# zeahmed/NeuralASR

Measured on AMD Instinct MI355X. Metric: audio-frames/sec (fwd+bwd+CTC+Adam) at batch 16 per GPU, higher is better.
Workload: dtype f32

## Files before the change

### neuralasr_amd/csrc/gemm.hip

```cpp
#include "kernels.h"

namespace nasr {

typedef float f32x16 __attribute__((ext_vector_type(16)));

constexpr int BM = 128, BN = 128, BK = 16, LDT = 132;

struct GemmParams {
  const float* A;
  const float* B;
  float* C;
  int M, N, K, lda, ldb, ldc;
  const int* a_map;
  int a_shift, a_rows;
  const int* c_map;
  const float* bias;
  int split_k, kchunk;
  float* slabs;
};

__device__ __forceinline__ int phys_row(const int* map, int shift, int rows, int logical) {
  int r = map ? map[logical] : logical + shift;
  return (r >= 0 && r < rows) ? r : -1;
}

__device__ __forceinline__ float4 ld4(const float* __restrict__ p) { return *reinterpret_cast<const float4*>(p); }
__device__ __forceinline__ float4 sel4(bool ok, float4 v) {
  return make_float4(ok ? v.x : 0.f, ok ? v.y : 0.f, ok ? v.z : 0.f, ok ? v.w : 0.f);
}

template <bool ACOL, bool BCOL>
__global__ __launch_bounds__(256, 2) void gemm_kernel(GemmParams p) {
  __shared__ __attribute__((aligned(16))) float As[2][BK][LDT];
  __shared__ __attribute__((aligned(16))) float Bs[2][BK][LDT];
  const int tid = threadIdx.x, lane = tid & 63, w = tid >> 6;
  const int m0 = blockIdx.y * BM, n0 = blockIdx.x * BN;
  const int kbeg = blockIdx.z * p.kchunk;
  const int kend = min(p.K, kbeg + p.kchunk);
  const int nk = (kend - kbeg + BK - 1) / BK;
  const float* __restrict__ Ag = p.A;
  const float* __restrict__ Bg = p.B;

  constexpr int NS = BK / 8, KQ = BK / 4;
  bool aok[NS], bok[NS];
  size_t ao[NS], bo[NS];
#pragma unroll
  for (int j = 0; j < NS; ++j) {
    const int idx = tid + 256 * j;
    const int r = idx / KQ, kq = idx % KQ, q = idx & 31;
    if (!ACOL) {
      const int pa = (m0 + r < p.M) ? phys_row(p.a_map, p.a_shift, p.a_rows, m0 + r) : -1;
      aok[j] = pa >= 0;
      ao[j] = aok[j] ? (size_t)pa * p.lda + 4 * kq : 0;
    } else {
      aok[j] = (m0 + 4 * q < p.M);
      ao[j] = aok[j] ? (size_t)(m0 + 4 * q) : 0;
    }
    if (BCOL) {
      bok[j] = n0 + r < p.N;
      bo[j] = bok[j] ? (size_t)(n0 + r) * p.ldb + 4 * kq : 0;
    } else {
      bok[j] = (n0 + 4 * q < p.N);
      bo[j] = bok[j] ? (size_t)(n0 + 4 * q) : 0;
    }
  }

  float4 ra[NS], rb[NS];
#define NASR_GLOAD(K0)                                                                              \
  _Pragma("unroll") for (int j = 0; j < NS; ++j) {                                                  \
    const int kk_ = (tid + 256 * j) >> 5;                                                           \
    const bool kr_ = (K0) + 4 * ((tid + 256 * j) % KQ) < kend, kc_ = (K0) + kk_ < kend;             \
    if (!ACOL) {                                                                                    \
      const bool o_ = aok[j] && kr_;                                                                \
      ra[j] = sel4(o_, ld4(Ag + (o_ ? ao[j] + (K0) : 0)));                                          \
    } else {                                                                                        \
      const int pr_ = kc_ ? phys_row(p.a_map, p.a_shift, p.a_rows, (K0) + kk_) : -1;                \
      const bool o_ = aok[j] && pr_ >= 0;                                                           \
      ra[j] = sel4(o_, ld4(Ag + (o_ ? (size_t)pr_ * p.lda + ao[j] : 0)));                           \
    }                                                                                               \
    if (BCOL) {                                                                                     \
      const bool o_ = bok[j] && kr_;                                                                \
      rb[j] = sel4(o_, ld4(Bg + (o_ ? bo[j] + (K0) : 0)));                                          \
    } else {                                                                                        \
      const bool o_ = bok[j] && kc_;                                                                \
      rb[j] = sel4(o_, ld4(Bg + (o_ ? (size_t)((K0) + kk_) * p.ldb + bo[j] : 0)));                  \
    }                                                                                               \
  }
#define NASR_LSTORE(BUF)                                                                            \
  _Pragma("unroll") for (int j = 0; j < NS; ++j) {                                                  \
    const int idx_ = tid + 256 * j;                                                                 \
    const int r_ = idx_ / KQ, kq_ = idx_ % KQ, kk_ = idx_ >> 5, q_ = idx_ & 31;                     \
    if (!ACOL) {                                                                                    \
      As[BUF][4 * kq_ + 0][r_] = ra[j].x; As[BUF][4 * kq_ + 1][r_] = ra[j].y;                       \
      As[BUF][4 * kq_ + 2][r_] = ra[j].z; As[BUF][4 * kq_ + 3][r_] = ra[j].w;                       \
    } else {                                                                                        \
      *reinterpret_cast<float4*>(&As[BUF][kk_][4 * q_]) = ra[j];                                    \
    }                                                                                               \
    if (BCOL) {                                                                                     \
      Bs[BUF][4 * kq_ + 0][r_] = rb[j].x; Bs[BUF][4 * kq_ + 1][r_] = rb[j].y;                       \
      Bs[BUF][4 * kq_ + 2][r_] = rb[j].z; Bs[BUF][4 * kq_ + 3][r_] = rb[j].w;                       \
    } else {                                                                                        \
      *reinterpret_cast<float4*>(&Bs[BUF][kk_][4 * q_]) = rb[j];                                    \
    }                                                                                               \
  }

  f32x16 acc00, acc01, acc10, acc11;
#pragma unroll
  for (int r = 0; r < 16; ++r) { acc00[r] = 0.f; acc01[r] = 0.f; acc10[r] = 0.f; acc11[r] = 0.f; }

  const int wm = (w >> 1) * 64, wn = (w & 1) * 64;
  const int li = lane & 31, lk = lane >> 5;

  if (nk > 0) {
    NASR_GLOAD(kbeg);
    NASR_LSTORE(0);
  }
  __syncthreads();
  for (int kt = 0; kt < nk; ++kt) {
    const int buf = kt & 1;
    const bool more = kt + 1 < nk;
    if (more) NASR_GLOAD(kbeg + (kt + 1) * BK);
    float a0 = As[buf][lk][wm + li], a1 = As[buf][lk][wm + 32 + li];
    float b0 = Bs[buf][lk][wn + li], b1 = Bs[buf][lk][wn + 32 + li];
#pragma unroll
    for (int ks = 0; ks < BK / 2; ++ks) {
      float na0 = 0.f, na1 = 0.f, nb0 = 0.f, nb1 = 0.f;
      if (ks + 1 < BK / 2) {
        const int k = 2 * (ks + 1) + lk;
        na0 = As[buf][k][wm + li]; na1 = As[buf][k][wm + 32 + li];
        nb0 = Bs[buf][k][wn + li]; nb1 = Bs[buf][k][wn + 32 + li];
      }
      acc00 = __builtin_amdgcn_mfma_f32_32x32x2f32(a0, b0, acc00, 0, 0, 0);
      acc01 = __builtin_amdgcn_mfma_f32_32x32x2f32(a0, b1, acc01, 0, 0, 0);
      acc10 = __builtin_amdgcn_mfma_f32_32x32x2f32(a1, b0, acc10, 0, 0, 0);
      acc11 = __builtin_amdgcn_mfma_f32_32x32x2f32(a1, b1, acc11, 0, 0, 0);
      a0 = na0; a1 = na1; b0 = nb0; b1 = nb1;
    }
    if (more) NASR_LSTORE(buf ^ 1);
    __syncthreads();
  }
#undef NASR_GLOAD
#undef NASR_LSTORE

#pragma unroll
  for (int t = 0; t < 4; ++t) {
    const int mi = t >> 1, ni = t & 1;
    const f32x16 acc = t == 0 ? acc00 : t == 1 ? acc01 : t == 2 ? acc10 : acc11;
    const int col = n0 + wn + 32 * ni + li;
    if (col >= p.N) continue;
    const float bv = (p.bias && p.split_k == 1) ? p.bias[col] : 0.f;
#pragma unroll
    for (int r = 0; r < 16; ++r) {
      const int row = m0 + wm + 32 * mi + (r & 3) + 8 * (r >> 2) + 4 * lk;
      if (row >= p.M) continue;
      if (p.split_k > 1) {
        p.slabs[((size_t)blockIdx.z * p.M + row) * p.N + col] = acc[r];
      } else {
        const int pr = p.c_map ? p.c_map[row] : row;
        if (pr >= 0) p.C[(size_t)pr * p.ldc + col] = acc[r] + bv;
      }
    }
  }
}

__global__ __launch_bounds__(256) void gemm_reduce_kernel(GemmParams p) {
  const int64_t n4 = (int64_t)p.M * p.N / 4;
  for (int64_t i = blockIdx.x * (int64_t)blockDim.x + threadIdx.x; i < n4; i += (int64_t)gridDim.x * blockDim.x) {
    const int64_t e = i * 4;
    const int row = (int)(e / p.N), col = (int)(e % p.N);
    float4 s = *reinterpret_cast<const float4*>(p.slabs + e);
    for (int k = 1; k < p.split_k; ++k) {
      const float4 v = *reinterpret_cast<const float4*>(p.slabs + (size_t)k * p.M * p.N + e);
      s.x += v.x; s.y += v.y; s.z += v.z; s.w += v.w;
    }
    if (p.bias) { s.x += p.bias[col]; s.y += p.bias[col + 1]; s.z += p.bias[col + 2]; s.w += p.bias[col + 3]; }
    const int pr = p.c_map ? p.c_map[row] : row;
    if (pr >= 0) *reinterpret_cast<float4*>(p.C + (size_t)pr * p.ldc + col) = s;
  }
}

int gemm_pick_split(int M, int N, int K) {
  const int tiles = ((M + BM - 1) / BM) * ((N + BN - 1) / BN);
  int s = (512 + tiles - 1) / tiles;
  const int max_s = K / 128;
  if (s > max_s) s = max_s;
  if (s < 1) s = 1;
  return s;
}

void launch_gemm(const GemmDesc& g, hipStream_t st) {
  GemmParams p;
  p.A = g.A; p.B = g.B; p.C = g.C;
  p.M = g.M; p.N = g.N; p.K = g.K; p.lda = g.lda; p.ldb = g.ldb; p.ldc = g.ldc;
  p.a_map = g.a_map; p.a_shift = g.a_shift; p.a_rows = g.a_rows; p.c_map = g.c_map; p.bias = g.bias;
  p.split_k = g.split_k < 1 ? 1 : g.split_k;
  p.slabs = g.slabs;
  int kt = (g.K + BK - 1) / BK;
  int per = (kt + p.split_k - 1) / p.split_k;
  p.kchunk = per * BK;
  p.split_k = (kt + per - 1) / per;
  dim3 grid((g.N + BN - 1) / BN, (g.M + BM - 1) / BM, p.split_k), block(256);
  if (!g.a_col && !g.b_col) hipLaunchKernelGGL((gemm_kernel<false, false>), grid, block, 0, st, p);
  else if (g.a_col && !g.b_col) hipLaunchKernelGGL((gemm_kernel<true, false>), grid, block, 0, st, p);
  else if (!g.a_col && g.b_col) hipLaunchKernelGGL((gemm_kernel<false, true>), grid, block, 0, st, p);
  else hipLaunchKernelGGL((gemm_kernel<true, true>), grid, block, 0, st, p);
  if (p.split_k > 1) {
    int64_t n4 = (int64_t)g.M * g.N / 4;
    int blocks = (int)((n4 + 255) / 256);
    if (blocks > 2048) blocks = 2048;
    hipLaunchKernelGGL(gemm_reduce_kernel, dim3(blocks), dim3(256), 0, st, p);
  }
}

}
```

### neuralasr_amd/csrc/kernels.h

```cpp
#pragma once
#include <hip/hip_runtime.h>
#include <stdint.h>

namespace nasr {

const char* test_hook(const char* name);

struct GemmDesc {
  const float* A;
  const float* B;
  float* C;
  int M, N, K;
  int lda, ldb, ldc;
  bool a_col;
  bool b_col;
  const int* a_map;
  int a_shift;
  int a_rows;
  const int* c_map;
  const float* bias;
  int split_k;
  float* slabs;
};
void launch_gemm(const GemmDesc& g, hipStream_t st);
int gemm_pick_split(int M, int N, int K);

int tp_split2_parts(int rows);
int gemm_tp_tile_rows(int M);
size_t tph_bytes(int rows, int K);
size_t tph_scale_ws_floats(int rows, int K);
void launch_tph_scales(const float* src, int rows, int K, int ld, float* row_scale, float* row_inv, float* col_scale,
                       float* col_inv, float* ws, hipStream_t st);
constexpr int TPH_MAX_JOBS = 16;
struct TphScaleJob { const float* src; int rows, K, ld; float *row_scale, *row_inv, *col_scale, *col_inv; };
size_t tph_scale_batch_ws_floats(const TphScaleJob* jobs, int n);
void launch_tph_scales_batch(const TphScaleJob* jobs, int n, float* ws, hipStream_t st);
void launch_tph_scales_from_parts(const float* rowpart, int nrp, int rows, float* row_scale, float* row_inv, const float* colpart,
                                  int ncp, int K, float* col_scale, float* col_inv, hipStream_t st);
void launch_fill(float* p, float v, int n, hipStream_t st);
void launch_tph_split2(const float* src, unsigned char* tpN, unsigned char* tpT, int rows, int K, int ld,
                       const float* row_scale, float rs, const float* col_scale, float cs, float* colpart, hipStream_t st,
                       const int* rowmap = nullptr, const int* rowmap2 = nullptr, int col2 = 0);
void launch_gather_rows(float* dst, const float* src, const int* map, int n, float fill, hipStream_t st);
struct GemmTPHDesc {
  const unsigned char* A;
  const unsigned char* B;
  float* C;
  int M, N, K;
  int nkbA, nkbB;
  int ldc;
  int a_kshift;
  const float* bias;
  const float* a_inv;
  const float* b_inv;
  int split_k;
  float* slabs;
  int tile_rows;
  int nbatch;
  size_t a_bstride, b_bstride;
  int64_t c_bstride, ainv_bstride, binv_bstride;
  int a_kshift1;
  bool side;
  const int* c_map;
};
hipError_t gemm_tph_prepare();
int gemm_tph_pick_split(int M, int N, int K, int nbatch = 1);
void launch_gemm_tph(const GemmTPHDesc& g, hipStream_t st);

struct LstmDims { int T, B, Bp, H, Hp, D; };
void launch_repack_u(const float* U, float* Uf, float* Ub, int Hp, hipStream_t st);
int lstm_bwd_partials(int Hp);
struct StepWindow {
  LstmDims dm;
  const float *Uf, *Ub;
  float *hstate, *partial, *dcstate;
  float *gates, *cbuf, *out;
  float* dg;
  const float* dout;
  const int* seq_len;
  float forget_bias;
  const float* c0;
};
void lstm_steps_fwd(const StepWindow& w, int s0, int s1, hipStream_t st);
void lstm_steps_bwd(const StepWindow& w, int s0, int s1, hipStream_t st);
struct StepLeft { float *partial, *dc; };
float* lstm_steps_dcin(const StepWindow& w, int s);
StepLeft lstm_steps_left(const StepWindow& w, int s);
constexpr int LA_MAX_SLOTS = 64;
struct LaSlots { int held[LA_MAX_SLOTS], n[LA_MAX_SLOTS], emit[LA_MAX_SLOTS]; };
void launch_stream_load_state(const float* state, float* himg, float* cimg, int S, int H, int Bp, int Hp, hipStream_t st, int D = 1);
void launch_stream_save_state(const float* out, const float* cbuf, const LaSlots& sl, float* state, int S, int H, int Bp, int DH,
                              hipStream_t st);

struct LcGeom { int C, W, K, T, Bp; };
__host__ __device__ inline int lc_last_window(int len, int C, int W) { return len <= W ? 0 : (len - W + C - 1) / C; }
__host__ __device__ inline int lc_window_rows(int len, int k, int C, int W) {
  if (len < 1 || k > lc_last_window(len, C, W)) return 0;
  return len - k * C < W ? len - k * C : W;
}
void launch_lc_load_carry(const float* out, const float* cbuf, const int* wlen, int k, const LcGeom& g, float* himg, float* cimg,
                          int Hp, int D, hipStream_t st);
void launch_lc_carry_out(const float* part, int np, const float* dcs, const int* wlen_k, float* drow, float* dcc, int Bp, int Hp,
                         int DH, hipStream_t st);
void launch_lc_carry_dc(float* dcin, const float* dcc, int n, hipStream_t st);

void launch_pack_feats(const float* feats_bm, float* X0, int B, int Bp, int T, int F, int Fp, hipStream_t st);
void launch_expand_context(const float* centre, const float* pad, const int* seq_len, float* X0, int B, int Bp, int T,
                           int ctx, int ncep, int Fp, hipStream_t st);
void launch_expand_context_masked(const float* centre, const float* pad, const int* seq_len, const int* masks, int nm,
                                  int static_width, float* X0, int B, int Bp, int T, int ctx, int ncep, int Fp,
                                  hipStream_t st);
void launch_la_window(const float* hold_in, const float* fresh, const LaSlots& sl, float* win, float* hold_out, int S, int R,
                      int Tc, int T, int rows, int F, hipStream_t st);
void launch_lc_gather(const float* src, const int* wlen, float* dst, const LcGeom& g, int F, hipStream_t st);
void launch_lc_emit(const float* outv, const int* seq_len, float* top, const LcGeom& g, int DH, hipStream_t st);
void launch_lc_scatter(const float* dtop, const int* seq_len, const int* wlen, float* doutv, const LcGeom& g, int DH,
                       hipStream_t st);

struct XcdCtl {
  unsigned xcc_count[8];
  unsigned error;
  unsigned pad[23];
};
static_assert(sizeof(XcdCtl) == 32 * sizeof(unsigned), "the control blocks' head is 32 words");
struct PersistCtl : XcdCtl {
  unsigned flags[8 * 128];
#if defined(NASR_PSTAMP) && NASR_PSTAMP
  unsigned stamps[256][12];
#endif
};
bool persist_supported(int Hp);
size_t persist_image_floats(int Hp, bool bwd);
size_t persist_xch_floats(int Hp);
size_t persist_hx_bytes(int Hp);
size_t persist_px_bytes();
hipError_t persist_prepare();
constexpr int PERSIST_MAX_MATS = 16;
void launch_repack_persist(const float* P, const int64_t* offs, int n, float* Upf, float* Upb, int Hp, const float* col_scale,
                           hipStream_t st);
void launch_lstm_persist_fwd(const LstmDims& dm, const float* Upf, const float* cinv, float* gates, float* cbuf,
                             float* out, const int* seq_len, float* xch, PersistCtl* ctl, unsigned* sticky, float* fault,
                             float forget_bias, hipStream_t st, bool ctl_zeroed = false);
void launch_lstm_persist_bwd(const LstmDims& dm, const float* Upb, const float* gates, float* dgbuf, const float* cbuf,
                             const float* dout, const int* seq_len, float* xch, PersistCtl* ctl, unsigned* sticky,
                             float* fault, hipStream_t st, bool ctl_zeroed = false, float* rowpart = nullptr,
                             float* colpart = nullptr, bool lean = false);
size_t persist_dgmax_floats(int T, int Bp, int Hp, int D);

struct WideCtl : XcdCtl {
  unsigned stamps[160];
};
struct WideGeom {
  int T, Bp, Hp, D, d;
  int inject;
  int scale_shift;
  float* fault;
};
bool wide_supported(int Hp, int Bp);
size_t wide_image_bytes(int Hp);
size_t wide_hx_bytes(int Bp);
size_t wide_part_bytes(int Bp);
hipError_t wide_prepare();
void launch_repack_wide(const float* U, const float* cs, void* Uw, int Hp, hipStream_t st);
void launch_lstm_wide_fwd(const LstmDims& dm, int d, const void* Uw, const float* cinv, float* gates, float* cbuf,
                          float* out, const int* seq_len, void* hx, float* part, WideCtl* ctl, unsigned* sticky,
                          float* fault, float forget_bias, hipStream_t st);

size_t wide_px_bytes(int Bp);
void launch_repack_wide_bwd(const float* U, const float* rs, void* Uwb, int Hp, hipStream_t st);
void launch_wide_row_scales(const LstmDims& dm, const float* dout, const int* seq_len, float* srow, hipStream_t st);
void launch_lstm_wide_bwd(const LstmDims& dm, int d, const void* Uwb, const float* rinv, const float* srow,
                          const float* gates, float* dgbuf, const float* cbuf, const float* dout, const int* seq_len,
                          float* inbox, void* px, WideCtl* ctl, unsigned* sticky, float* fault, hipStream_t st);

void launch_dense_act(float* z, int R, int Bp, int B, int W, int ld, float clip, float p, uint32_t seed, uint32_t counter,
                      int stage, hipStream_t st);
void launch_dense_act_bwd(float* dy, const float* y, int64_t n, float clip, float p, hipStream_t st);

struct CtcDims {
  int Tp;
  int B, Bp, C, Cp, Lmax;
  int KS;
  int Tws;
  float* lprobs = nullptr;
  double* goff = nullptr;
};
constexpr int ctc_states_per_lane(int Lmax) {
  const int KS = (2 * (Lmax > 0 ? Lmax : 0) + 1 + 63) / 64;
  return KS <= 1 ? 2 : KS <= 8 ? KS : KS <= 12 ? 12 : KS <= 16 ? 16 : KS;
}
constexpr int ctc_group_rows(int Tws) { return Tws / 4 + 3; }
void launch_ctc_logz(const CtcDims& d, const float* logits, const int* seq_len, float* logz, hipStream_t st);
void launch_ctc_alpha_beta(const CtcDims& d, const float* logits, const float* logz, const int* labels,
                           const int* label_len, const int* seq_len, float* alpha, float* beta, double* aoff,
                           double* boff, float* nll, double* logp, hipStream_t st);
void launch_ctc_grad(const CtcDims& d, float* logits, const float* logz, const int* label_len, const int* seq_len,
                     const int* cstart, const int* cpos, const float* alpha, const float* beta, const double* aoff,
                     const double* boff, const double* logp, float scale, hipStream_t st);
void launch_mean(const float* v, int n, float* out, hipStream_t st);
void launch_greedy(const CtcDims& d, const float* logits, const int* seq_len, int* argmax_ws, int* ids, int* lens,
                   hipStream_t st);

bool ctc_align_bp_in_lds(int F, int L);
size_t ctc_align_ws_words(int B, int F, int L);
int launch_ctc_align(const CtcDims& d, int F, const float* logits, const float* logz, const int* labels, const int* label_len,
                     const int* seq_len, unsigned* bpws, int* path, double* score, hipStream_t st);

void launch_distill_rows(const CtcDims& d, const float* student, const float* teacher, const int* seq_len, float weight,
                         float tau, float* dgrad, float* klrow, double* kd, hipStream_t st);
void launch_distill_combine(const double* kd, int B, float weight, float tau, float* loss, float* parts,
                            const float* teacher_fault, float* fault, hipStream_t st);
void launch_distill_add(const CtcDims& d, float* grad, const float* dgrad, hipStream_t st);

struct AdamDev { long long step; float lr_t; int applied; };
struct EmaDev { long long updates; float omd; };
constexpr int ADAM_MAX_BLOCKS = 2048;
void launch_adam(float* p, float* m, float* v, const float* g, int64_t n, AdamDev* state, float lr, float beta1, float beta2,
                 float eps, float gscale, const float* fault, float* e, EmaDev* ema, float decay, hipStream_t st);
void launch_swap16(float* a, float* b, int64_t n, hipStream_t st);
struct ClipDev { double last_norm; float last_coef, s; int skip, pad; double window_max_norm; long long steps, clipped, skipped; };
constexpr int GRAD_SUMSQ_MAX_BLOCKS = 1024;
int grad_sumsq_blocks(int64_t n);
void launch_adam_clipped(float* p, float* m, float* v, const float* g, int64_t n, AdamDev* state, ClipDev* clip, double* part,
                         float lr, float beta1, float beta2, float eps, float gscale, float max_norm, const float* fault,
                         float* e, EmaDev* ema, float decay, hipStream_t st);
void launch_colsum(const float* M, int R, int N, int ld, float* out, float* ws, hipStream_t st);
void launch_colsum_parts(const float* part, int nparts, int N, float* out, hipStream_t st);
void launch_reduce_slabs(const float* slabs, int S, int64_t n, float* out, hipStream_t st);
void launch_reduce_slabs_rows(const float* slabs, int S, int M, int N, int ldc, const int* map, float* out, hipStream_t st);
void launch_ring_standin(float* buf, int64_t n, int nblocks, int passes, hipStream_t st);

}
```

### neuralasr_amd/csrc/optim.hip

```cpp
#include "kernels.h"

#include <cstdlib>

namespace nasr {

const char* test_hook(const char* name) {
  static const bool enabled = [] {
    const char* e = getenv("NASR_TEST_HOOKS");
    return e && e[0] == '1';
  }();
  return enabled ? getenv(name) : nullptr;
}

__device__ __forceinline__ void adam_advance(AdamDev* st, float lr, float b1, float b2) {
  const long long t = st->step + 1;
  st->step = t;
  st->lr_t = (float)((double)lr * sqrt(1.0 - pow((double)b2, (double)t)) / (1.0 - pow((double)b1, (double)t)));
  st->applied = 1;
}

__device__ __forceinline__ void ema_advance(EmaDev* em, float decay) {
  if (!em) return;
  const long long n = em->updates;
  const double ramp = (1.0 + (double)n) / (10.0 + (double)n);
  const double d = (double)decay < ramp ? (double)decay : ramp;
  em->omd = (float)(1.0 - d);
  em->updates = n + 1;
}

__global__ void adam_prepare_kernel(AdamDev* st, const float* __restrict__ fault, float lr, float b1, float b2, EmaDev* em,
                                    float decay) {
  if (fault && *fault != 0.f) {
    st->applied = 0;
    return;
  }
  adam_advance(st, lr, b1, b2);
  ema_advance(em, decay);
}

#define NASR_ADAM_SWEEP(EMA)                                                                                              \
  for (int64_t i = blockIdx.x * (int64_t)blockDim.x + threadIdx.x; i < n4; i += (int64_t)gridDim.x * blockDim.x) {       \
    float4 gg = reinterpret_cast<const float4*>(g)[i];                                                                    \
    float4 mm = reinterpret_cast<float4*>(m)[i];                                                                          \
    float4 vv = reinterpret_cast<float4*>(v)[i];                                                                          \
    float4 pp = reinterpret_cast<float4*>(p)[i];                                                                          \
    NASR_ADAM1(x) NASR_ADAM1(y) NASR_ADAM1(z) NASR_ADAM1(w)                                                               \
    reinterpret_cast<float4*>(m)[i] = mm;                                                                                 \
    reinterpret_cast<float4*>(v)[i] = vv;                                                                                 \
    reinterpret_cast<float4*>(p)[i] = pp;                                                                                 \
    NASR_EMA_##EMA                                                                                                        \
  }
#define NASR_EMA_0
#define NASR_EMA_1                                                                                                        \
  {                                                                                                                       \
    float4 ee = reinterpret_cast<float4*>(e)[i];                                                                          \
    ee.x = fmaf(omd, pp.x - ee.x, ee.x);                                                                                  \
    ee.y = fmaf(omd, pp.y - ee.y, ee.y);                                                                                  \
    ee.z = fmaf(omd, pp.z - ee.z, ee.z);                                                                                  \
    ee.w = fmaf(omd, pp.w - ee.w, ee.w);                                                                                  \
    reinterpret_cast<float4*>(e)[i] = ee;                                                                                 \
  }
#define NASR_ADAM1(c)                                   \
  {                                                     \
    const float gc = gg.c * gscale;                     \
    mm.c = b1 * mm.c + (1.f - b1) * gc;                 \
    vv.c = b2 * vv.c + (1.f - b2) * gc * gc;            \
    pp.c = pp.c - lr_t * mm.c / (sqrtf(vv.c) + eps);    \
  }

__global__ __launch_bounds__(256) void adam_kernel(float* __restrict__ p, float* __restrict__ m, float* __restrict__ v,
                                                   const float* __restrict__ g, int64_t n4, const AdamDev* __restrict__ st,
                                                   float b1, float b2, float eps, float gscale,
                                                   const float* __restrict__ fault) {
  if (fault && *fault != 0.f) return;
  const float lr_t = st->lr_t;
  NASR_ADAM_SWEEP(0)
}

__global__ __launch_bounds__(256) void adam_ema_kernel(float* __restrict__ p, float* __restrict__ m, float* __restrict__ v,
                                                       const float* __restrict__ g, float* __restrict__ e, int64_t n4,
                                                       const AdamDev* __restrict__ st, const EmaDev* __restrict__ em, float b1,
                                                       float b2, float eps, float gscale, const float* __restrict__ fault) {
  if (fault && *fault != 0.f) return;
  const float lr_t = st->lr_t;
  const float omd = em->omd;
  NASR_ADAM_SWEEP(1)
}

__global__ __launch_bounds__(256) void adam_clip_kernel(float* __restrict__ p, float* __restrict__ m, float* __restrict__ v,
                                                        const float* __restrict__ g, int64_t n4,
                                                        const AdamDev* __restrict__ st, const ClipDev* __restrict__ clip,
                                                        float b1, float b2, float eps, const float* __restrict__ fault) {
  if (fault && *fault != 0.f) return;
  if (clip->skip) return;
  const float lr_t = st->lr_t;
  const float gscale = clip->s;
  NASR_ADAM_SWEEP(0)
}

__global__ __launch_bounds__(256) void adam_clip_ema_kernel(float* __restrict__ p, float* __restrict__ m, float* __restrict__ v,
                                                            const float* __restrict__ g, float* __restrict__ e, int64_t n4,
                                                            const AdamDev* __restrict__ st, const ClipDev* __restrict__ clip,
                                                            const EmaDev* __restrict__ em, float b1, float b2, float eps,
                                                            const float* __restrict__ fault) {
  if (fault && *fault != 0.f) return;
  if (clip->skip) return;
  const float lr_t = st->lr_t;
  const float gscale = clip->s;
  const float omd = em->omd;
  NASR_ADAM_SWEEP(1)
}
#undef NASR_ADAM1
#undef NASR_EMA_0
#undef NASR_EMA_1
#undef NASR_ADAM_SWEEP

__global__ __launch_bounds__(256) void swap16_kernel(float4* __restrict__ a, float4* __restrict__ b, int64_t n4) {
  for (int64_t i = blockIdx.x * (int64_t)blockDim.x + threadIdx.x; i < n4; i += (int64_t)gridDim.x * blockDim.x) {
    const float4 x = a[i], y = b[i];
    a[i] = y;
    b[i] = x;
  }
}

__device__ __forceinline__ double block_sum_fixed(double a, double* sm) {
#pragma unroll
  for (int off = 32; off > 0; off >>= 1) a += __shfl_down(a, off, 64);
  if ((threadIdx.x & 63) == 0) sm[threadIdx.x >> 6] = a;
  __syncthreads();
  return (sm[0] + sm[1]) + (sm[2] + sm[3]);
}

int grad_sumsq_blocks(int64_t n) {
  const int64_t b = (n / 4 + 255) / 256;
  return b < 1 ? 1 : b > GRAD_SUMSQ_MAX_BLOCKS ? GRAD_SUMSQ_MAX_BLOCKS : (int)b;
}

__global__ __launch_bounds__(256) void grad_sumsq_part_kernel(const float* __restrict__ g, int64_t n,
                                                              double* __restrict__ part, const float* __restrict__ fault) {
  __shared__ double sm[4];
  if (fault && *fault != 0.f) return;
  const int64_t n4 = n / 4;
  const int64_t per = (n4 + gridDim.x - 1) / gridDim.x;
  const int64_t lo = per * blockIdx.x, hi = lo + per < n4 ? lo + per : n4;
  double ax = 0.0, ay = 0.0, az = 0.0, aw = 0.0;
#pragma unroll 4
  for (int64_t i = lo + threadIdx.x; i < hi; i += 256) {
    const float4 v = reinterpret_cast<const float4*>(g)[i];
    ax += (double)v.x * (double)v.x;
    ay += (double)v.y * (double)v.y;
    az += (double)v.z * (double)v.z;
    aw += (double)v.w * (double)v.w;
  }
  if (blockIdx.x == 0 && threadIdx.x == 0)
    for (int64_t i = n4 * 4; i < n; ++i) ax += (double)g[i] * (double)g[i];
  const double s = block_sum_fixed((ax + ay) + (az + aw), sm);
  if (threadIdx.x == 0) part[blockIdx.x] = s;
}

__global__ __launch_bounds__(256) void grad_clip_final_kernel(const double* __restrict__ part, int nparts, ClipDev* clip,
                                                              AdamDev* st, const float* __restrict__ fault, float gscale,
                                                              float max_norm, float lr, float b1, float b2, EmaDev* em,
                                                              float decay) {
  __shared__ double sm[4];
  if (fault && *fault != 0.f) {
    if (threadIdx.x == 0) st->applied = 0;
    return;
  }
  double a = 0.0;
  for (int k = threadIdx.x; k < nparts; k += 256) a += part[k];
  const double n2 = block_sum_fixed(a, sm);
  if (threadIdx.x != 0) return;
  const double norm = fabs((double)gscale) * sqrt(n2);
  clip->last_norm = norm;
  if (!isfinite(norm)) {
    clip->skip = 1;
    clip->skipped += 1;
    st->applied = 0;
    return;
  }
  const float coef = (float)(norm > (double)max_norm ? (double)max_norm / norm : 1.0);
  clip->skip = 0;
  clip->s = gscale * coef;
  clip->last_coef = coef;
  clip->steps += 1;
  if (coef < 1.f) clip->clipped += 1;
  if (norm > clip->window_max_norm) clip->window_max_norm = norm;
  adam_advance(st, lr, b1, b2);
  ema_advance(em, decay);
}

void launch_adam(float* p, float* m, float* v, const float* g, int64_t n, AdamDev* state, float lr, float beta1, float beta2,
                 float eps, float gscale, const float* fault, float* e, EmaDev* ema, float decay, hipStream_t st) {
  const int64_t n4 = n / 4;
  int blocks = (int)((n4 + 255) / 256);
  if (blocks > ADAM_MAX_BLOCKS) blocks = ADAM_MAX_BLOCKS;
  hipLaunchKernelGGL(adam_prepare_kernel, dim3(1), dim3(1), 0, st, state, fault, lr, beta1, beta2, e ? ema : nullptr, decay);
  if (e)
    hipLaunchKernelGGL(adam_ema_kernel, dim3(blocks), dim3(256), 0, st, p, m, v, g, e, n4, state, ema, beta1, beta2, eps, gscale,
                       fault);
  else
    hipLaunchKernelGGL(adam_kernel, dim3(blocks), dim3(256), 0, st, p, m, v, g, n4, state, beta1, beta2, eps, gscale, fault);
}

void launch_swap16(float* a, float* b, int64_t n, hipStream_t st) {
  const int64_t n4 = n / 4;
  int blocks = (int)((n4 + 255) / 256);
  if (blocks > ADAM_MAX_BLOCKS) blocks = ADAM_MAX_BLOCKS;
  hipLaunchKernelGGL(swap16_kernel, dim3(blocks), dim3(256), 0, st, reinterpret_cast<float4*>(a), reinterpret_cast<float4*>(b), n4);
}

void launch_adam_clipped(float* p, float* m, float* v, const float* g, int64_t n, AdamDev* state, ClipDev* clip, double* part,
                         float lr, float beta1, float beta2, float eps, float gscale, float max_norm, const float* fault,
                         float* e, EmaDev* ema, float decay, hipStream_t st) {
  const int64_t n4 = n / 4;
  int blocks = (int)((n4 + 255) / 256);
  if (blocks > ADAM_MAX_BLOCKS) blocks = ADAM_MAX_BLOCKS;
  const int nparts = grad_sumsq_blocks(n);
  hipLaunchKernelGGL(grad_sumsq_part_kernel, dim3(nparts), dim3(256), 0, st, g, n, part, fault);
  hipLaunchKernelGGL(grad_clip_final_kernel, dim3(1), dim3(256), 0, st, part, nparts, clip, state, fault, gscale, max_norm, lr,
                     beta1, beta2, e ? ema : nullptr, decay);
  if (e)
    hipLaunchKernelGGL(adam_clip_ema_kernel, dim3(blocks), dim3(256), 0, st, p, m, v, g, e, n4, state, clip, ema, beta1, beta2,
                       eps, fault);
  else
    hipLaunchKernelGGL(adam_clip_kernel, dim3(blocks), dim3(256), 0, st, p, m, v, g, n4, state, clip, beta1, beta2, eps, fault);
}

constexpr int CS_SPLIT = 32;

__global__ __launch_bounds__(256) void colsum_part_kernel(const float* __restrict__ M, int R, int N, int ld,
                                                          float* __restrict__ part) {
  __shared__ float sm[4][64];
  const int cx = threadIdx.x & 63, ry = threadIdx.x >> 6;
  const int n = blockIdx.x * 64 + cx;
  const int rs = blockIdx.y;
  const int per = (R + CS_SPLIT - 1) / CS_SPLIT;
  const int r0 = rs * per, r1 = min(R, r0 + per);
  float s = 0.f;
  if (n < N)
    for (int r = r0 + ry; r < r1; r += 4) s += M[(size_t)r * ld + n];
  sm[ry][cx] = s;
  __syncthreads();
  if (ry == 0 && n < N) part[(size_t)rs * N + n] = (sm[0][cx] + sm[1][cx]) + (sm[2][cx] + sm[3][cx]);
}

__global__ __launch_bounds__(256) void colsum_final_kernel(const float* __restrict__ part, int nparts, int N,
                                                           float* __restrict__ out) {
  __shared__ float sm[16][17];
  const int cx = threadIdx.x & 15, q = threadIdx.x >> 4;
  const int n = blockIdx.x * 16 + cx;
  float s = 0.f;
  if (n < N)
    for (int k = q; k < nparts; k += 16) s += part[(size_t)k * N + n];
  sm[q][cx] = s;
  __syncthreads();
  if (q == 0 && n < N) {
    float t = 0.f;
#pragma unroll
    for (int i = 0; i < 16; ++i) t += sm[i][cx];
    out[n] = t;
  }
}

void launch_colsum_parts(const float* part, int nparts, int N, float* out, hipStream_t st) {
  hipLaunchKernelGGL(colsum_final_kernel, dim3((N + 15) / 16), dim3(256), 0, st, part, nparts, N, out);
}

void launch_colsum(const float* M, int R, int N, int ld, float* out, float* ws, hipStream_t st) {
  hipLaunchKernelGGL(colsum_part_kernel, dim3((N + 63) / 64, CS_SPLIT), dim3(256), 0, st, M, R, N, ld, ws);
  launch_colsum_parts(ws, CS_SPLIT, N, out, st);
}

__global__ __launch_bounds__(256) void reduce_slabs_kernel(const float* __restrict__ slabs, int S, int64_t n,
                                                           float* __restrict__ out) {
  for (int64_t i = blockIdx.x * (int64_t)blockDim.x + threadIdx.x; i < n; i += (int64_t)gridDim.x * blockDim.x) {
    float s = slabs[i];
    for (int k = 1; k < S; ++k) s += slabs[(size_t)k * n + i];
    out[i] = s;
  }
}
void launch_reduce_slabs(const float* slabs, int S, int64_t n, float* out, hipStream_t st) {
  int blocks = (int)((n + 255) / 256);
  if (blocks > 2048) blocks = 2048;
  hipLaunchKernelGGL(reduce_slabs_kernel, dim3(blocks), dim3(256), 0, st, slabs, S, n, out);
}

__global__ __launch_bounds__(256) void reduce_slabs_rows_kernel(const float* __restrict__ slabs, int S, int M, int N, int ldc,
                                                                const int* __restrict__ map, float* __restrict__ out) {
  const int64_t n4 = (int64_t)M * N / 4, per = (int64_t)M * N;
  for (int64_t i = blockIdx.x * (int64_t)256 + threadIdx.x; i < n4; i += (int64_t)gridDim.x * 256) {
    const int m = (int)(i * 4 / N), c = (int)(i * 4 % N);
    const int orow = map[m];
    if (orow < 0) continue;
    float4 a = *reinterpret_cast<const float4*>(slabs + i * 4);
    for (int s = 1; s < S; ++s) {
      const float4 b = *reinterpret_cast<const float4*>(slabs + s * per + i * 4);
      a.x += b.x; a.y += b.y; a.z += b.z; a.w += b.w;
    }
    *reinterpret_cast<float4*>(out + (size_t)orow * ldc + c) = a;
  }
}
void launch_reduce_slabs_rows(const float* slabs, int S, int M, int N, int ldc, const int* map, float* out, hipStream_t st) {
  int blocks = (int)(((int64_t)M * N / 4 + 255) / 256);
  if (blocks > 2048) blocks = 2048;
  hipLaunchKernelGGL(reduce_slabs_rows_kernel, dim3(blocks), dim3(256), 0, st, slabs, S, M, N, ldc, map, out);
}

__global__ __launch_bounds__(256) void ring_standin_kernel(float4* __restrict__ buf, long long n4, int passes) {
  const long long per = (n4 + gridDim.x - 1) / gridDim.x;
  const long long lo = per * blockIdx.x, hi = lo + per < n4 ? lo + per : n4;
  for (int p = 0; p < passes; ++p)
    for (long long i = lo + threadIdx.x; i < hi; i += 256) {
      float4 v = buf[i];
      v.x *= 1.f; v.y *= 1.f; v.z *= 1.f; v.w *= 1.f;
      asm volatile("" : "+v"(v.x), "+v"(v.y), "+v"(v.z), "+v"(v.w));
      buf[i] = v;
    }
}

void launch_ring_standin(float* buf, int64_t n, int nblocks, int passes, hipStream_t st) {
  hipLaunchKernelGGL(ring_standin_kernel, dim3(nblocks), dim3(256), 0, st, reinterpret_cast<float4*>(buf), (long long)(n / 4), passes);
}

}
```

Measured before the change: 1.298 million.

## Add narrow-N GEMM tile, specialized epilogue stores, and unrolled slab reductions

Adds a 128x32 GEMM tile variant for N<=32 so small-output GEMMs stop wasting three quarters of a 128-wide tile, and makes the epilogue compile-time specialized for plain, mapped and slab stores with a full-tile fast path. Replaces the split-K reduce kernel with the shared reduce_slabs_rows kernel, which now also applies the bias. Both slab reduction kernels are templated on the slab count with several float4 vectors per thread, unrolled loads issued up front, and a CU-scaled grid size. The cost is more template instantiations, longer compile times and higher register pressure.

```diff
diff --git a/neuralasr_amd/csrc/gemm.hip b/neuralasr_amd/csrc/gemm.hip
--- a/neuralasr_amd/csrc/gemm.hip
+++ b/neuralasr_amd/csrc/gemm.hip
@@ -1,3 +1,5 @@
+#include <type_traits>
+
 #include "kernels.h"
 
 namespace nasr {
@@ -5,6 +7,7 @@
 typedef float f32x16 __attribute__((ext_vector_type(16)));
 
 constexpr int BM = 128, BN = 128, BK = 16, LDT = 132;
+constexpr int BN_NARROW = 32;
 
 struct GemmParams {
   const float* A;
@@ -29,12 +32,15 @@
   return make_float4(ok ? v.x : 0.f, ok ? v.y : 0.f, ok ? v.z : 0.f, ok ? v.w : 0.f);
 }
 
-template <bool ACOL, bool BCOL>
+template <bool ACOL, bool BCOL, int TN_>
 __global__ __launch_bounds__(256, 2) void gemm_kernel(GemmParams p) {
+  constexpr bool WIDE = TN_ == BN;
+  constexpr int FM = WIDE ? 2 : 1, FN = WIDE ? 2 : 1;
+  constexpr int LDB = TN_ + 4, QN = TN_ / 4;
   __shared__ __attribute__((aligned(16))) float As[2][BK][LDT];
-  __shared__ __attribute__((aligned(16))) float Bs[2][BK][LDT];
+  __shared__ __attribute__((aligned(16))) float Bs[2][BK][LDB];
   const int tid = threadIdx.x, lane = tid & 63, w = tid >> 6;
-  const int m0 = blockIdx.y * BM, n0 = blockIdx.x * BN;
+  const int m0 = blockIdx.y * BM, n0 = blockIdx.x * TN_;
   const int kbeg = blockIdx.z * p.kchunk;
   const int kend = min(p.K, kbeg + p.kchunk);
   const int nk = (kend - kbeg + BK - 1) / BK;
@@ -42,8 +48,10 @@
   const float* __restrict__ Bg = p.B;
 
   constexpr int NS = BK / 8, KQ = BK / 4;
-  bool aok[NS], bok[NS];
-  size_t ao[NS], bo[NS];
+  constexpr int NSB = WIDE ? NS : 1;
+  const bool bact = WIDE || tid < TN_ * KQ;
+  bool aok[NS], bok[NSB];
+  size_t ao[NS], bo[NSB];
 #pragma unroll
   for (int j = 0; j < NS; ++j) {
     const int idx = tid + 256 * j;
@@ -56,16 +64,21 @@
       aok[j] = (m0 + 4 * q < p.M);
       ao[j] = aok[j] ? (size_t)(m0 + 4 * q) : 0;
     }
+  }
+#pragma unroll
+  for (int j = 0; j < NSB; ++j) {
+    const int idx = tid + 256 * j;
+    const int r = idx / KQ, kq = idx % KQ, q = idx % QN;
     if (BCOL) {
-      bok[j] = n0 + r < p.N;
+      bok[j] = bact && n0 + r < p.N;
       bo[j] = bok[j] ? (size_t)(n0 + r) * p.ldb + 4 * kq : 0;
     } else {
-      bok[j] = (n0 + 4 * q < p.N);
+      bok[j] = bact && (n0 + 4 * q < p.N);
       bo[j] = bok[j] ? (size_t)(n0 + 4 * q) : 0;
     }
   }
 
-  float4 ra[NS], rb[NS];
+  float4 ra[NS], rb[NSB];
 #define NASR_GLOAD(K0)                                                                              \
   _Pragma("unroll") for (int j = 0; j < NS; ++j) {                                                  \
     const int kk_ = (tid + 256 * j) >> 5;                                                           \
@@ -78,12 +91,18 @@
       const bool o_ = aok[j] && pr_ >= 0;                                                           \
       ra[j] = sel4(o_, ld4(Ag + (o_ ? (size_t)pr_ * p.lda + ao[j] : 0)));                           \
     }                                                                                               \
-    if (BCOL) {                                                                                     \
-      const bool o_ = bok[j] && kr_;                                                                \
-      rb[j] = sel4(o_, ld4(Bg + (o_ ? bo[j] + (K0) : 0)));                                          \
-    } else {                                                                                        \
-      const bool o_ = bok[j] && kc_;                                                                \
-      rb[j] = sel4(o_, ld4(Bg + (o_ ? (size_t)((K0) + kk_) * p.ldb + bo[j] : 0)));                  \
+  }                                                                                                 \
+  if (bact) {                                                                                       \
+    _Pragma("unroll") for (int j = 0; j < NSB; ++j) {                                               \
+      const int kk_ = (tid + 256 * j) / QN;                                                         \
+      const bool kr_ = (K0) + 4 * ((tid + 256 * j) % KQ) < kend, kc_ = (K0) + kk_ < kend;           \
+      if (BCOL) {                                                                                   \
+        const bool o_ = bok[j] && kr_;                                                              \
+        rb[j] = sel4(o_, ld4(Bg + (o_ ? bo[j] + (K0) : 0)));                                        \
+      } else {                                                                                      \
+        const bool o_ = bok[j] && kc_;                                                              \
+        rb[j] = sel4(o_, ld4(Bg + (o_ ? (size_t)((K0) + kk_) * p.ldb + bo[j] : 0)));                \
+      }                                                                                             \
     }                                                                                               \
   }
 #define NASR_LSTORE(BUF)                                                                            \
@@ -96,19 +115,29 @@
     } else {                                                                                        \
       *reinterpret_cast<float4*>(&As[BUF][kk_][4 * q_]) = ra[j];                                    \
     }                                                                                               \
-    if (BCOL) {                                                                                     \
-      Bs[BUF][4 * kq_ + 0][r_] = rb[j].x; Bs[BUF][4 * kq_ + 1][r_] = rb[j].y;                       \
-      Bs[BUF][4 * kq_ + 2][r_] = rb[j].z; Bs[BUF][4 * kq_ + 3][r_] = rb[j].w;                       \
-    } else {                                                                                        \
-      *reinterpret_cast<float4*>(&Bs[BUF][kk_][4 * q_]) = rb[j];                                    \
-    }                                                                                               \
-  }
-
-  f32x16 acc00, acc01, acc10, acc11;
-#pragma unroll
-  for (int r = 0; r < 16; ++r) { acc00[r] = 0.f; acc01[r] = 0.f; acc10[r] = 0.f; acc11[r] = 0.f; }
-
-  const int wm = (w >> 1) * 64, wn = (w & 1) * 64;
+  }                                                                                                 \
+  if (bact) {                                                                                       \
+    _Pragma("unroll") for (int j = 0; j < NSB; ++j) {                                               \
+      const int idx_ = tid + 256 * j;                                                               \
+      const int r_ = idx_ / KQ, kq_ = idx_ % KQ, kk_ = idx_ / QN, q_ = idx_ % QN;                   \
+      if (BCOL) {                                                                                   \
+        Bs[BUF][4 * kq_ + 0][r_] = rb[j].x; Bs[BUF][4 * kq_ + 1][r_] = rb[j].y;                     \
+        Bs[BUF][4 * kq_ + 2][r_] = rb[j].z; Bs[BUF][4 * kq_ + 3][r_] = rb[j].w;                     \
+      } else {                                                                                      \
+        *reinterpret_cast<float4*>(&Bs[BUF][kk_][4 * q_]) = rb[j];                                  \
+      }                                                                                             \
+    }                                                                                               \
+  }
+
+  f32x16 acc[FM][FN];
+#pragma unroll
+  for (int i = 0; i < FM; ++i)
+#pragma unroll
+    for (int j = 0; j < FN; ++j)
+#pragma unroll
+      for (int r = 0; r < 16; ++r) acc[i][j][r] = 0.f;
+
+  const int wm = WIDE ? (w >> 1) * 64 : w * 32, wn = WIDE ? (w & 1) * 64 : 0;
   const int li = lane & 31, lk = lane >> 5;
 
   if (nk > 0) {
@@ -120,21 +149,33 @@
     const int buf = kt & 1;
     const bool more = kt + 1 < nk;
     if (more) NASR_GLOAD(kbeg + (kt + 1) * BK);
-    float a0 = As[buf][lk][wm + li], a1 = As[buf][lk][wm + 32 + li];
-    float b0 = Bs[buf][lk][wn + li], b1 = Bs[buf][lk][wn + 32 + li];
+    float a[FM], b[FN];
+#pragma unroll
+    for (int i = 0; i < FM; ++i) a[i] = As[buf][lk][wm + 32 * i + li];
+#pragma unroll
+    for (int j = 0; j < FN; ++j) b[j] = Bs[buf][lk][wn + 32 * j + li];
 #pragma unroll
     for (int ks = 0; ks < BK / 2; ++ks) {
-      float na0 = 0.f, na1 = 0.f, nb0 = 0.f, nb1 = 0.f;
+      float na[FM], nb[FN];
+#pragma unroll
+      for (int i = 0; i < FM; ++i) na[i] = 0.f;
+#pragma unroll
+      for (int j = 0; j < FN; ++j) nb[j] = 0.f;
       if (ks + 1 < BK / 2) {
         const int k = 2 * (ks + 1) + lk;
-        na0 = As[buf][k][wm + li]; na1 = As[buf][k][wm + 32 + li];
-        nb0 = Bs[buf][k][wn + li]; nb1 = Bs[buf][k][wn + 32 + li];
+#pragma unroll
+        for (int i = 0; i < FM; ++i) na[i] = As[buf][k][wm + 32 * i + li];
+#pragma unroll
+        for (int j = 0; j < FN; ++j) nb[j] = Bs[buf][k][wn + 32 * j + li];
       }
-      acc00 = __builtin_amdgcn_mfma_f32_32x32x2f32(a0, b0, acc00, 0, 0, 0);
-      acc01 = __builtin_amdgcn_mfma_f32_32x32x2f32(a0, b1, acc01, 0, 0, 0);
-      acc10 = __builtin_amdgcn_mfma_f32_32x32x2f32(a1, b0, acc10, 0, 0, 0);
-      acc11 = __builtin_amdgcn_mfma_f32_32x32x2f32(a1, b1, acc11, 0, 0, 0);
-      a0 = na0; a1 = na1; b0 = nb0; b1 = nb1;
+#pragma unroll
+      for (int i = 0; i < FM; ++i)
+#pragma unroll
+        for (int j = 0; j < FN; ++j) acc[i][j] = __builtin_amdgcn_mfma_f32_32x32x2f32(a[i], b[j], acc[i][j], 0, 0, 0);
+#pragma unroll
+      for (int i = 0; i < FM; ++i) a[i] = na[i];
+#pragma unroll
+      for (int j = 0; j < FN; ++j) b[j] = nb[j];
     }
     if (more) NASR_LSTORE(buf ^ 1);
     __syncthreads();
@@ -142,41 +183,62 @@
 #undef NASR_GLOAD
 #undef NASR_LSTORE
 
-#pragma unroll
-  for (int t = 0; t < 4; ++t) {
-    const int mi = t >> 1, ni = t & 1;
-    const f32x16 acc = t == 0 ? acc00 : t == 1 ? acc01 : t == 2 ? acc10 : acc11;
-    const int col = n0 + wn + 32 * ni + li;
-    if (col >= p.N) continue;
-    const float bv = (p.bias && p.split_k == 1) ? p.bias[col] : 0.f;
-#pragma unroll
-    for (int r = 0; r < 16; ++r) {
-      const int row = m0 + wm + 32 * mi + (r & 3) + 8 * (r >> 2) + 4 * lk;
-      if (row >= p.M) continue;
-      if (p.split_k > 1) {
-        p.slabs[((size_t)blockIdx.z * p.M + row) * p.N + col] = acc[r];
-      } else {
-        const int pr = p.c_map ? p.c_map[row] : row;
-        if (pr >= 0) p.C[(size_t)pr * p.ldc + col] = acc[r] + bv;
+  const int row0 = m0 + wm + 4 * lk, col0 = n0 + wn + li;
+  float bvv[FN];
+#pragma unroll
+  for (int ni = 0; ni < FN; ++ni) {
+    const int col = min(col0 + 32 * ni, p.N - 1);
+    bvv[ni] = (p.bias && p.split_k == 1) ? p.bias[col] : 0.f;
+  }
+  auto store_tile = [&](auto mode_c, auto full_c) {
+    constexpr int MODE = decltype(mode_c)::value;
+    constexpr bool FULL = decltype(full_c)::value;
+    float* const out = MODE == 2 ? p.slabs + (size_t)blockIdx.z * p.M * p.N : p.C;
+    const size_t ld = MODE == 2 ? (size_t)p.N : (size_t)p.ldc;
+    int orow[16];
+    auto load_rows = [&](int mi) {
+      if constexpr (MODE == 1) {
+#pragma unroll
+        for (int r = 0; r < 16; ++r) {
+          const int row = row0 + 32 * mi + (r & 3) + 8 * (r >> 2);
+          orow[r] = p.c_map[FULL ? row : min(row, p.M - 1)];
+        }
       }
-    }
-  }
-}
-
-__global__ __launch_bounds__(256) void gemm_reduce_kernel(GemmParams p) {
-  const int64_t n4 = (int64_t)p.M * p.N / 4;
-  for (int64_t i = blockIdx.x * (int64_t)blockDim.x + threadIdx.x; i < n4; i += (int64_t)gridDim.x * blockDim.x) {
-    const int64_t e = i * 4;
-    const int row = (int)(e / p.N), col = (int)(e % p.N);
-    float4 s = *reinterpret_cast<const float4*>(p.slabs + e);
-    for (int k = 1; k < p.split_k; ++k) {
-      const float4 v = *reinterpret_cast<const float4*>(p.slabs + (size_t)k * p.M * p.N + e);
-      s.x += v.x; s.y += v.y; s.z += v.z; s.w += v.w;
-    }
-    if (p.bias) { s.x += p.bias[col]; s.y += p.bias[col + 1]; s.z += p.bias[col + 2]; s.w += p.bias[col + 3]; }
-    const int pr = p.c_map ? p.c_map[row] : row;
-    if (pr >= 0) *reinterpret_cast<float4*>(p.C + (size_t)pr * p.ldc + col) = s;
-  }
+    };
+#pragma unroll
+    for (int mi = 0; mi < FM; ++mi) {
+      load_rows(mi);
+      asm volatile("" ::: "memory");
+#pragma unroll
+      for (int ni = 0; ni < FN; ++ni) {
+        const int col = col0 + 32 * ni;
+        if (!FULL && col >= p.N) continue;
+        const float bv = bvv[ni];
+#pragma unroll
+        for (int r = 0; r < 16; ++r) {
+          const int row = row0 + 32 * mi + (r & 3) + 8 * (r >> 2);
+          if (!FULL && row >= p.M) continue;
+          if constexpr (MODE == 2) {
+            out[(size_t)row * ld + col] = acc[mi][ni][r];
+          } else if constexpr (MODE == 1) {
+            if (orow[r] >= 0) out[(size_t)orow[r] * ld + col] = acc[mi][ni][r] + bv;
+          } else {
+            out[(size_t)row * ld + col] = acc[mi][ni][r] + bv;
+          }
+        }
+      }
+      asm volatile("" ::: "memory");
+    }
+  };
+  const bool full = m0 + wm + 32 * FM <= p.M && n0 + wn + 32 * FN <= p.N;
+  using T = std::true_type;
+  using F = std::false_type;
+  using Plain = std::integral_constant<int, 0>;
+  using Mapped = std::integral_constant<int, 1>;
+  using Slab = std::integral_constant<int, 2>;
+  if (p.split_k > 1) { if (full) store_tile(Slab{}, T{}); else store_tile(Slab{}, F{}); }
+  else if (p.c_map) { if (full) store_tile(Mapped{}, T{}); else store_tile(Mapped{}, F{}); }
+  else { if (full) store_tile(Plain{}, T{}); else store_tile(Plain{}, F{}); }
 }
 
 int gemm_pick_split(int M, int N, int K) {
@@ -186,6 +248,15 @@
   if (s > max_s) s = max_s;
   if (s < 1) s = 1;
   return s;
+}
+
+template <int TN_>
+static void launch_gemm_tile(const GemmDesc& g, const GemmParams& p, hipStream_t st) {
+  dim3 grid((g.N + TN_ - 1) / TN_, (g.M + BM - 1) / BM, p.split_k), block(256);
+  if (!g.a_col && !g.b_col) hipLaunchKernelGGL((gemm_kernel<false, false, TN_>), grid, block, 0, st, p);
+  else if (g.a_col && !g.b_col) hipLaunchKernelGGL((gemm_kernel<true, false, TN_>), grid, block, 0, st, p);
+  else if (!g.a_col && g.b_col) hipLaunchKernelGGL((gemm_kernel<false, true, TN_>), grid, block, 0, st, p);
+  else hipLaunchKernelGGL((gemm_kernel<true, true, TN_>), grid, block, 0, st, p);
 }
 
 void launch_gemm(const GemmDesc& g, hipStream_t st) {
@@ -199,17 +270,9 @@
   int per = (kt + p.split_k - 1) / p.split_k;
   p.kchunk = per * BK;
   p.split_k = (kt + per - 1) / per;
-  dim3 grid((g.N + BN - 1) / BN, (g.M + BM - 1) / BM, p.split_k), block(256);
-  if (!g.a_col && !g.b_col) hipLaunchKernelGGL((gemm_kernel<false, false>), grid, block, 0, st, p);
-  else if (g.a_col && !g.b_col) hipLaunchKernelGGL((gemm_kernel<true, false>), grid, block, 0, st, p);
-  else if (!g.a_col && g.b_col) hipLaunchKernelGGL((gemm_kernel<false, true>), grid, block, 0, st, p);
-  else hipLaunchKernelGGL((gemm_kernel<true, true>), grid, block, 0, st, p);
-  if (p.split_k > 1) {
-    int64_t n4 = (int64_t)g.M * g.N / 4;
-    int blocks = (int)((n4 + 255) / 256);
-    if (blocks > 2048) blocks = 2048;
-    hipLaunchKernelGGL(gemm_reduce_kernel, dim3(blocks), dim3(256), 0, st, p);
-  }
-}
-
-}
+  if (g.N <= BN_NARROW) launch_gemm_tile<BN_NARROW>(g, p, st);
+  else launch_gemm_tile<BN>(g, p, st);
+  if (p.split_k > 1) launch_reduce_slabs_rows(p.slabs, p.split_k, g.M, g.N, g.ldc, g.c_map, g.C, st, g.bias);
+}
+
+}
diff --git a/neuralasr_amd/csrc/kernels.h b/neuralasr_amd/csrc/kernels.h
--- a/neuralasr_amd/csrc/kernels.h
+++ b/neuralasr_amd/csrc/kernels.h
@@ -227,7 +227,8 @@
 void launch_colsum(const float* M, int R, int N, int ld, float* out, float* ws, hipStream_t st);
 void launch_colsum_parts(const float* part, int nparts, int N, float* out, hipStream_t st);
 void launch_reduce_slabs(const float* slabs, int S, int64_t n, float* out, hipStream_t st);
-void launch_reduce_slabs_rows(const float* slabs, int S, int M, int N, int ldc, const int* map, float* out, hipStream_t st);
+void launch_reduce_slabs_rows(const float* slabs, int S, int M, int N, int ldc, const int* map, float* out, hipStream_t st,
+                              const float* bias = nullptr);
 void launch_ring_standin(float* buf, int64_t n, int nblocks, int passes, hipStream_t st);
 
 }
diff --git a/neuralasr_amd/csrc/optim.hip b/neuralasr_amd/csrc/optim.hip
--- a/neuralasr_amd/csrc/optim.hip
+++ b/neuralasr_amd/csrc/optim.hip
@@ -1,6 +1,7 @@
 #include "kernels.h"
 
 #include <cstdlib>
+#include <type_traits>
 
 namespace nasr {
 
@@ -272,39 +273,165 @@
   launch_colsum_parts(ws, CS_SPLIT, N, out, st);
 }
 
-__global__ __launch_bounds__(256) void reduce_slabs_kernel(const float* __restrict__ slabs, int S, int64_t n,
+__device__ __forceinline__ void add4(float4& a, const float4& b) { a.x += b.x; a.y += b.y; a.z += b.z; a.w += b.w; }
+
+template <int S, int V>
+__device__ __forceinline__ void slab_sum(const float4* (&src)[V], int64_t per4, int Srt, float4 (&acc)[V]) {
+  constexpr int C = S > 0 ? S : 8;
+  float4 x[C][V];
+#pragma unroll
+  for (int k = 0; k < C; ++k)
+#pragma unroll
+    for (int v = 0; v < V; ++v) x[k][v] = src[v][k * per4];
+#pragma unroll
+  for (int v = 0; v < V; ++v) acc[v] = x[0][v];
+#pragma unroll
+  for (int k = 1; k < C; ++k)
+#pragma unroll
+    for (int v = 0; v < V; ++v) add4(acc[v], x[k][v]);
+  if constexpr (S == 0) {
+    int k = 8;
+    for (; k + 8 <= Srt; k += 8) {
+#pragma unroll
+      for (int j = 0; j < 8; ++j)
+#pragma unroll
+        for (int v = 0; v < V; ++v) x[j][v] = src[v][(k + j) * per4];
+#pragma unroll
+      for (int j = 0; j < 8; ++j)
+#pragma unroll
+        for (int v = 0; v < V; ++v) add4(acc[v], x[j][v]);
+    }
+    for (; k < Srt; ++k) {
+#pragma unroll
+      for (int v = 0; v < V; ++v) x[0][v] = src[v][k * per4];
+#pragma unroll
+      for (int v = 0; v < V; ++v) add4(acc[v], x[0][v]);
+    }
+  }
+}
+
+constexpr int slab_vecs(int S) { return S == 1 ? 8 : S == 2 ? 4 : 2; }
+
+static int slab_blocks(int64_t nvec, int V) {
+  static int cus = 0;
+  if (cus == 0) {
+    int dev = 0, n = 0;
+    if (hipGetDevice(&dev) != hipSuccess || hipDeviceGetAttribute(&n, hipDeviceAttributeMultiprocessorCount, dev) != hipSuccess || n < 1)
+      n = 256;
+    cus = n;
+  }
+  const int64_t want = (nvec + 256 * V - 1) / (256 * V);
+  return (int)(want < 1 ? 1 : want > 8 * cus ? 8 * cus : want);
+}
+
+template <int S, int V>
+__global__ __launch_bounds__(256) void reduce_slabs_kernel(const float* __restrict__ slabs, int Srt, int64_t n,
                                                            float* __restrict__ out) {
+  const int64_t n4 = n / 4, step = (int64_t)gridDim.x * (256 * V);
+  const float4* __restrict__ s4 = reinterpret_cast<const float4*>(slabs);
+  float4* __restrict__ o4 = reinterpret_cast<float4*>(out);
+  int64_t i = blockIdx.x * (int64_t)(256 * V) + threadIdx.x;
+  for (; i + 256 * (V - 1) < n4; i += step) {
+    const float4* src[V];
+    float4 acc[V];
+#pragma unroll
+    for (int v = 0; v < V; ++v) src[v] = s4 + i + 256 * v;
+    slab_sum<S, V>(src, n4, Srt, acc);
+#pragma unroll
+    for (int v = 0; v < V; ++v) o4[i + 256 * v] = acc[v];
+  }
+  for (int v = 0; v < V - 1; ++v) {
+    const int64_t j = i + 256 * v;
+    if (j >= n4) break;
+    const float4* src[1] = {s4 + j};
+    float4 acc[1];
+    slab_sum<S, 1>(src, n4, Srt, acc);
+    o4[j] = acc[0];
+  }
+}
+
+__global__ __launch_bounds__(256) void reduce_slabs_scalar_kernel(const float* __restrict__ slabs, int S, int64_t n,
+                                                                  float* __restrict__ out) {
   for (int64_t i = blockIdx.x * (int64_t)blockDim.x + threadIdx.x; i < n; i += (int64_t)gridDim.x * blockDim.x) {
     float s = slabs[i];
     for (int k = 1; k < S; ++k) s += slabs[(size_t)k * n + i];
     out[i] = s;
   }
 }
+
+static bool aligned16(const void* p) { return (reinterpret_cast<uintptr_t>(p) & 15) == 0; }
+
+template <typename F>
+static void with_slab_count(int S, F&& f) {
+  switch (S) {
+    case 1: f(std::integral_constant<int, 1>{}); break;
+    case 2: f(std::integral_constant<int, 2>{}); break;
+    case 3: f(std::integral_constant<int, 3>{}); break;
+    case 4: f(std::integral_constant<int, 4>{}); break;
+    case 5: f(std::integral_constant<int, 5>{}); break;
+    case 6: f(std::integral_constant<int, 6>{}); break;
+    case 7: f(std::integral_constant<int, 7>{}); break;
+    case 8: f(std::integral_constant<int, 8>{}); break;
+    default: f(std::integral_constant<int, 0>{}); break;
+  }
+}
+
 void launch_reduce_slabs(const float* slabs, int S, int64_t n, float* out, hipStream_t st) {
-  int blocks = (int)((n + 255) / 256);
-  if (blocks > 2048) blocks = 2048;
-  hipLaunchKernelGGL(reduce_slabs_kernel, dim3(blocks), dim3(256), 0, st, slabs, S, n, out);
-}
-
-__global__ __launch_bounds__(256) void reduce_slabs_rows_kernel(const float* __restrict__ slabs, int S, int M, int N, int ldc,
-                                                                const int* __restrict__ map, float* __restrict__ out) {
-  const int64_t n4 = (int64_t)M * N / 4, per = (int64_t)M * N;
-  for (int64_t i = blockIdx.x * (int64_t)256 + threadIdx.x; i < n4; i += (int64_t)gridDim.x * 256) {
-    const int m = (int)(i * 4 / N), c = (int)(i * 4 % N);
-    const int orow = map[m];
-    if (orow < 0) continue;
-    float4 a = *reinterpret_cast<const float4*>(slabs + i * 4);
-    for (int s = 1; s < S; ++s) {
-      const float4 b = *reinterpret_cast<const float4*>(slabs + s * per + i * 4);
-      a.x += b.x; a.y += b.y; a.z += b.z; a.w += b.w;
+  if (n <= 0 || S < 1) return;
+  if (n % 4 != 0 || !aligned16(slabs) || !aligned16(out)) {
+    int blocks = (int)((n + 255) / 256);
+    if (blocks > 2048) blocks = 2048;
+    hipLaunchKernelGGL(reduce_slabs_scalar_kernel, dim3(blocks), dim3(256), 0, st, slabs, S, n, out);
+    return;
+  }
+  with_slab_count(S, [&](auto sc) {
+    constexpr int SC = decltype(sc)::value, V = slab_vecs(SC);
+    hipLaunchKernelGGL((reduce_slabs_kernel<SC, V>), dim3(slab_blocks(n / 4, V)), dim3(256), 0, st, slabs, S, n, out);
+  });
+}
+
+template <int S, int V>
+__global__ __launch_bounds__(256) void reduce_slabs_rows_kernel(const float* __restrict__ slabs, int Srt, int M, int N, int ldc,
+                                                                const int* __restrict__ map, const float* __restrict__ bias,
+                                                                float* __restrict__ out) {
+  const int64_t n4 = (int64_t)M * N / 4, step = (int64_t)gridDim.x * (256 * V);
+  const bool small = n4 < (1 << 29);
+  const float4* __restrict__ s4 = reinterpret_cast<const float4*>(slabs);
+  for (int64_t i = blockIdx.x * (int64_t)(256 * V) + threadIdx.x; i < n4; i += step) {
+    const float4* src[V];
+    float4 acc[V];
+    int64_t dst[V];
+    int col[V];
+#pragma unroll
+    for (int v = 0; v < V; ++v) {
+      const int64_t j = i + 256 * v;
+      const int64_t e = j < n4 ? j * 4 : 0;
+      int m, c;
+      if (small) { m = (int)((uint32_t)e / (uint32_t)N); c = (int)((uint32_t)e % (uint32_t)N); }
+      else { m = (int)(e / N); c = (int)(e % N); }
+      const int orow = map ? map[m] : m;
+      const bool ok = j < n4 && orow >= 0;
+      src[v] = s4 + (ok ? e / 4 : 0);
+      dst[v] = ok ? (int64_t)orow * ldc + c : -1;
+      col[v] = c;
     }
-    *reinterpret_cast<float4*>(out + (size_t)orow * ldc + c) = a;
-  }
-}
-void launch_reduce_slabs_rows(const float* slabs, int S, int M, int N, int ldc, const int* map, float* out, hipStream_t st) {
-  int blocks = (int)(((int64_t)M * N / 4 + 255) / 256);
-  if (blocks > 2048) blocks = 2048;
-  hipLaunchKernelGGL(reduce_slabs_rows_kernel, dim3(blocks), dim3(256), 0, st, slabs, S, M, N, ldc, map, out);
+    slab_sum<S, V>(src, n4, Srt, acc);
+#pragma unroll
+    for (int v = 0; v < V; ++v) {
+      if (bias) { acc[v].x += bias[col[v]]; acc[v].y += bias[col[v] + 1]; acc[v].z += bias[col[v] + 2]; acc[v].w += bias[col[v] + 3]; }
+      if (dst[v] >= 0) *reinterpret_cast<float4*>(out + dst[v]) = acc[v];
+    }
+  }
+}
+
+void launch_reduce_slabs_rows(const float* slabs, int S, int M, int N, int ldc, const int* map, float* out, hipStream_t st,
+                              const float* bias) {
+  if (M <= 0 || N <= 0 || S < 1) return;
+  with_slab_count(S, [&](auto sc) {
+    constexpr int SC = decltype(sc)::value, V = slab_vecs(SC);
+    hipLaunchKernelGGL((reduce_slabs_rows_kernel<SC, V>), dim3(slab_blocks((int64_t)M * N / 4, V)), dim3(256), 0, st, slabs, S, M, N,
+                       ldc, map, bias, out);
+  });
 }
 
 __global__ __launch_bounds__(256) void ring_standin_kernel(float4* __restrict__ buf, long long n4, int passes) {
```

Measured after the change: 1.306 million, median of 6. About the same (+0.6%).
